# yeyupiaoling/PPASR

Hardware: AMD Instinct MI355X
Metric: audio-seconds/s (RTF^-1) Conformer-streaming fbank, batch32 per GPU, ctc_greedy (higher is better)
Workload: dtype f32; 1 GPU; configs[1]: Conformer streaming (configs/conformer.yml), fbank-80, 32 x 10 s utterances per GPU, V=4233, ctc_greedy, features resident in HBM -> token ids + scores on device; global_batch=32, frames=1000, decoder=ctc_greedy, parallelism=utterance-dp1, pipelined=False, gemm=f32

## Files before the change

### ppasr_amd/csrc/conformer_kernels.hip

```cpp
#include <cstdlib>

#include "conformer_kernels.h"
#include "launch.h"
#include "phases.h"
#include "h3.h"

#include <math.h>

namespace ppasr {
#ifdef PPASR_PHASE_TS
}
extern "C" __attribute__((visibility("default"))) int ppasr_debug_read_phase_ts(long long* out) {
  return (int)hipMemcpyFromSymbol(out, HIP_SYMBOL(ppasr::g_phase_ts), sizeof(long long) * 128);
}
extern "C" __attribute__((visibility("default"))) int ppasr_debug_read_wave_ts(long long* out) {
  return (int)hipMemcpyFromSymbol(out, HIP_SYMBOL(ppasr::g_wave_ts), sizeof(long long) * 512);
}
extern "C" __attribute__((visibility("default"))) int ppasr_debug_read_wg_ts(long long* out) {
  return (int)hipMemcpyFromSymbol(out, HIP_SYMBOL(ppasr::g_wg_ts), sizeof(long long) * 2 * 1024);
}
namespace ppasr {
#endif


// ... 281 lines not shown
    }
    const float bval = w.pw1_b[col];
    const float bgate = w.pw1_b[kD + col];
#pragma unroll
    for (int r = 0; r < 16; ++r) {
      int row = acc_row(r, lane);
      float val = av[0][0][r] + bval;
      float gate = ag[0][0][r] + bgate;
      if (row < valid) g[(size_t)(r0 + row) * kD + col] = val * sigmoidf(gate);
    }
  }
}
template <bool H3>
__global__ __launch_bounds__(kThreads) void k_pw1_glu_cols(const float* __restrict__ xhat, float* __restrict__ g, LayerW w,
                                                           int M, PadSkip ps) {
  extern __shared__ __attribute__((aligned(16))) float smem[];
  const int blk = pad_block_of(ps, kRows, M);
  if (blk < 0) return;
  float* bufA = smem;
  float* vals = bufA + kRows * kLda + (H3 ? 128 : 0);
  const int lane = lane_id(), wave = wave_id();
  const int r0 = blk * kRows;
  const int valid = min(kRows, M - r0);
  const int is_gate = wave >> 2, t = wave & 3, y = blockIdx.y;
  const int col = 128 * y + 32 * t + (lane & 31);
  const f32x4* seg = w.pw1 + (size_t)((is_gate ? 8 : 0) + 4 * y + t) * kTs256;
  BRing<1> ring;
  ring_prime(ring, seg, 0);
  rb_load_rows(bufA, kLda, xhat + (size_t)r0 * kD, kRows, valid);
  __syncthreads();
  f32x16 acc[1][1];
  acc_zero(acc);
  if constexpr (H3) unit_std_h3(bufA, seg, nullptr, ring, acc);
  else rb_gemm<1, 1, kG256>(bufA, kLda, seg, 0, nullptr, 0, ring, acc);
  const float bv = w.pw1_b[(is_gate ? kD : 0) + col];
  if (!is_gate) {
#pragma unroll
    for (int r = 0; r < 16; ++r) vals[acc_row(r, lane) * 132 + 32 * t + (lane & 31)] = acc[0][0][r] + bv;
  }
  __syncthreads();
  if (is_gate) {
#pragma unroll
    for (int r = 0; r < 16; ++r) {
      const int row = acc_row(r, lane);
      if (row < valid) g[(size_t)(r0 + row) * kD + col] = vals[row * 132 + 32 * t + (lane & 31)] * sigmoidf(acc[0][0][r] + bv);
    }
  }
}
constexpr size_t kLdsOutGlu = 2 * kRows * kLda * sizeof(float);
constexpr size_t kLdsPw1Cols = (kRows * kLda + kRows * 132) * sizeof(float);
void launch_out_glu(const float* ctx, const float* x1, float* x2, float* g, float* xhat_out, const LayerW& w,
                    const int64_t* lens, int M, int Tp, int mask_mul, hipStream_t st, const PadSkip& ps, float* split_xhat,
                    bool h3, HistMove* hm, int rows) {
  check_form("launch_out_glu", rows, h3 || xhat_out || split_xhat || hm);
  if (rows == 16) return LayerStagesT<16>::out_glu(ctx, x1, x2, g, w, lens, M, Tp, mask_mul, st, ps);
  if (rows == kW16) return LayerStagesT<kW16>::out_glu(ctx, x1, x2, g, w, lens, M, Tp, mask_mul, st, ps);
  float* xh = xhat_out ? xhat_out : split_xhat;
  if (split_xhat && !h3 && M <= kSplitRows16Max && !ps.tab) {
    const bool move = hm && hm->hist && hm->lo > 0 && hm->lo <= 30;
    launch_out_glu_split_16(ctx, x1, x2, g, xh, w, lens, M, Tp, mask_mul, st, ps, move ? hm->hist : nullptr, move ? hm->lo : 0);
    if (move) hm->done = true;
    return;
  }
  const dim3 grid((M + kRows - 1) / kRows);
  if (h3)
    PPASR_LAUNCH(k_out_glu<true>, grid, dim3(kThreads), kLdsOutGlu + 512, st, ctx, x1, x2, g, xh, w, lens, M, Tp, mask_mul, ps,
                 split_xhat ? 1 : 0);
  else
    PPASR_LAUNCH(k_out_glu<false>, grid, dim3(kThreads), kLdsOutGlu, st, ctx, x1, x2, g, xh, w, lens, M, Tp, mask_mul, ps,
                 split_xhat ? 1 : 0);
  if (split_xhat) {
    if (h3)
      PPASR_LAUNCH(k_pw1_glu_cols<true>, dim3(grid.x, 2), dim3(kThreads), kLdsPw1Cols + 512, st, xh, g, w, M, ps);
    else
      PPASR_LAUNCH(k_pw1_glu_cols<false>, dim3(grid.x, 2), dim3(kThreads), kLdsPw1Cols, st, xh, g, w, M, ps);
  }
}

constexpr int kPLd = 68;
constexpr int kPTile = 32 * kPLd;
constexpr int kFusedAttnFloats = kWaves * kPTile + kWaves * 64 + kRows * kLda;
static_assert(2 * kRows * kLda <= kWaves * kPTile + kWaves * 64, "bufX/bufA alias the attention scratch");
static_assert(kRows * kLda + 128 + 4 * kPTile <= kWaves * kPTile, "the d rows (fp16 x3: the Q'_v planes, 512 B longer) and the four merge tiles fit in front of Stat");
static_assert(kH3TileBytes <= kRows * kLda * 4 + 512, "fp16 x3: the Q'_u planes at bufC run 512 B past it (the launch asks for them)");
static_assert(kRows * kLda * 4 + kH3TileBytes <= kWaves * kPTile * 4, "fp16 x3: operand planes at bufA stay in front of Stat");
static_assert(kFusedAttnFloats * 4 <= 160 * 1024, "LDS budget");
template <bool H3>
__device__ __forceinline__ void attn_out_glu_body(const AttnArgs& a, int B, const float* __restrict__ x1, float* __restrict__ x2,
                                                  float* __restrict__ g, const LayerW& w) {
  extern __shared__ __attribute__((aligned(16))) float smem[];
  float* Ps = smem;
  float* Stat = Ps + kWaves * kPTile;
  float* bufC = Stat + kWaves * 64;
  float* bufX = smem;
  float* bufA = bufX + kRows * kLda;
  const int lane = lane_id(), wave = wave_id();
  const int h = wave >> 1, khalf = wave & 1;
  const int nq = (a.T1 + 31) / 32;
  const int slot = blockIdx.x >> 3;
  const int b = (slot / nq) * 8 + (blockIdx.x & 7);
  const int q0 = (slot % nq) * 32;
  if (b >= B) return;
  const int T = a.T1;
  const int valid = min(32, T - q0);
  const float* __restrict__ qb = a.q + (size_t)b * T * a.q_stride;
  const float* __restrict__ kbp = a.k + (size_t)b * a.T2 * a.k_stride;
  const float* __restrict__ vbp = a.v + (size_t)b * a.T2 * a.v_stride;
  const float* __restrict__ ptab = a.ptab + (size_t)a.pos0 * kD;
  const int pstride = a.pos_stride;
  const int64_t len_b = a.lens ? a.lens[b] : (int64_t)a.mask_mul * a.T2;
  int T2 = a.T2;
  if (a.pad_skip > 0 && a.lens) {
    const int64_t lb = len_b > 0 ? len_b : 0;
    const int64_t n_valid = (lb + a.mask_mul - 1) / a.mask_mul;
    if (q0 >= min((int64_t)T, n_valid + (a.pad_skip - 1))) return;
    T2 = (int)max((int64_t)1, min((int64_t)T2, n_valid));
  }
  float* QV = Ps;
  float* P = Ps + kRows * kLda + (H3 ? 128 : 0) + (wave >> 1) * kPTile;
  BRing<1> ring;
  const f32x4* seg_o = w.wo + (size_t)wave * kTs256;
  const f32x4* seg_val = w.pw1 + (size_t)wave * kTs256;
  const f32x4* seg_gate = w.pw1 + (size_t)(8 + wave) * kTs256;
  const int hh = lane >> 5, l31 = lane & 31;
  constexpr int NG = H3 ? 16 : 8;
  PPASR_TS(32);
  PPASR_WG_TS(512 + 0);

  const int mrow0 = b * T;
  const int shift = mrow0 & 7;
  int kv_end = (int)min((int64_t)T2, max((int64_t)0, (len_b + a.mask_mul - 1) / a.mask_mul));
  const int U = kv_end > 0 ? kv_end + shift : 0;
  constexpr float kScale = 0.125f * 1.4426950408889634f * (H3 ? 1.0f / (kH3Sa * kH3Sa) : 1.0f);
  const __amdgpu_buffer_rsrc_t rs_k = wstream_rsrc(kbp + h * (H3 ? 32 : 64)), rs_p = wstream_rsrc(ptab + h * (H3 ? 32 : 64)),
                               rs_v = wstream_rsrc(a.vt + ((size_t)(2 * h) * (a.vt_stride >> 3) + ((mrow0 - shift) >> 3)) * 256);
  const int voff_v = lane * 16;
  const int kstride_b = a.k_stride * 4, pstride_b = pstride * kD * 4;
  int vk[2], vp[2];
  auto key_offsets = [&](int u0) {
#pragma unroll
    for (int t = 0; t < 2; ++t) {
      const int key = min(max(u0 - shift + 32 * t + l31, 0), kv_end - 1);
      vk[t] = key * kstride_b + 16 * hh;
      if constexpr (H3) vp[t] = key * pstride_b + 16 * hh;
    }
  };
  constexpr int NKB = H3 ? 4 : 2;
  f32x4 kq[NKB][4][2];
  auto load_sg = [&](int buf, int sg) {
#pragma unroll
    for (int i = 0; i < 4; ++i) {
      if constexpr (H3) {
        const int soff = (sg & 1) * 512 + 32 * i;
        kq[buf][i][0] = sg < 2 ? wstream_load(rs_k, vk[0], soff) : wstream_load(rs_p, vp[0], soff);
        kq[buf][i][1] = sg < 2 ? wstream_load(rs_k, vk[1], soff) : wstream_load(rs_p, vp[1], soff);
      } else {
        kq[buf][i][0] = wstream_load(rs_k, vk[0], (4 * sg + i) * 32);
        kq[buf][i][1] = wstream_load(rs_k, vk[1], (4 * sg + i) * 32);
      }
    }
  };
  auto prime_k = [&](int u0) {
    key_offsets(u0);
    load_sg(0, 0);
    if constexpr (H3) load_sg(1, 1);
  };

  const float* __restrict__ dtab = a.dtab ? a.dtab + (size_t)h * a.dtab_len + a.pos0 : nullptr;
  {
    if constexpr (!H3) attn_stage_d(Ps + h * kDRow, dtab, khalf * 64 + lane, shift, U <= kDRow ? U : 0, pstride);
    const f32x4 pu = *reinterpret_cast<const f32x4*>(a.pos_u + 4 * lane), pv = *reinterpret_cast<const f32x4*>(a.pos_v + 4 * lane);
    bool bad = false;
    for (int row = wave; row < kRows; row += kWaves) {
      f32x4 v = {0.f, 0.f, 0.f, 0.f};
      if (row < valid) v = *reinterpret_cast<const f32x4*>(qb + (size_t)(q0 + row) * a.q_stride + 4 * lane);
      if constexpr (H3) {
        f16x4 hi, lo;
        h3_split4((v + pu) * kH3Sa, hi, lo, bad);
        _Float16* pu_pl = reinterpret_cast<_Float16*>(bufC) + row * kLdh + 4 * lane;
        *reinterpret_cast<f16x4*>(pu_pl) = hi;
        *reinterpret_cast<f16x4*>(pu_pl + kPlaneH) = lo;
        h3_split4((v + pv) * kH3Sa, hi, lo, bad);
        _Float16* pv_pl = reinterpret_cast<_Float16*>(QV) + row * kLdh + 4 * lane;
        *reinterpret_cast<f16x4*>(pv_pl) = hi;
        *reinterpret_cast<f16x4*>(pv_pl + kPlaneH) = lo;
      } else {
        *reinterpret_cast<f32x4*>(bufC + row * kLda + 4 * lane) = v + pu;
      }
    }
    if constexpr (H3) h3_note(bad);
    __syncthreads();
  }
  const float* qfrag_u = bufC + l31 * kLda + h * 64 + 4 * hh;
  auto qfrag = [&](int gk) -> f32x4 { return *reinterpret_cast<const f32x4*>(qfrag_u + 8 * gk); };
  PPASR_TS(33);
  if (khalf * 128 < U) prime_k(khalf * 128);
  f32x16 acc_o[2];
#pragma unroll
  for (int t = 0; t < 2; ++t)
#pragma unroll
    for (int r = 0; r < 16; ++r) acc_o[t][r] = 0.f;
  float m_run = -INFINITY, l_run = 0.f;
  bool first = true;

  const int nkb = (U + 255) / 256;
  for (int kb = 0; kb < nkb; ++kb) {
    for (int sb = 0; sb < 2; ++sb) {
      const int u0 = kb * 256 + khalf * 128 + sb * 64;
      if (u0 >= U) break;
      int u_next = sb == 0 ? u0 + 64 : (kb + 1) * 256 + khalf * 128;
      if (u_next >= U) u_next = (sb == 0 && (kb + 1) * 256 + khalf * 128 < U) ? (kb + 1) * 256 + khalf * 128 : -1;
      const bool edge = (u0 < shift) || (u0 + 64 > U);
      if (kb == 0) PPASR_WAVE_TS(16 + 4 * sb);
      const int soff_v = (u0 >> 3) * 1024, soff_v1 = soff_v + (a.vt_stride >> 3) * 1024;
      auto vload = [&](int q, int ct) -> f32x4 { return wstream_load(rs_v, voff_v, (ct ? soff_v1 : soff_v) + q * 1024); };
      constexpr int PQ = 8;
      f32x4 ringv[PQ][2];
      auto prime_v = [&]() {
#pragma unroll
        for (int q = 0; q < PQ; ++q) {
          ringv[q][0] = vload(q, 0);
          ringv[q][1] = vload(q, 1);
        }
      };
      f32x16 acc_s[2];
      if constexpr (H3) {
#pragma unroll
        for (int t = 0; t < 2; ++t)
#pragma unroll
          for (int r = 0; r < 16; ++r) acc_s[t][r] = 0.f;
      } else {
        attn_score_init(acc_s, U <= kDRow ? Ps + h * kDRow + u0 + 4 * hh : nullptr, dtab, u0 - shift + 4 * hh, kv_end, pstride);
      }
      if constexpr (H3) {
        const _Float16* qu = reinterpret_cast<const _Float16*>(bufC) + l31 * kLdh + h * 64 + 8 * hh;
        const _Float16* qv = reinterpret_cast<const _Float16*>(QV) + l31 * kLdh + h * 64 + 8 * hh;
        load_sg(2, 2);
        load_sg(3, 3);
#pragma unroll
        for (int sg = 0; sg < 4; ++sg) {
          const _Float16* qp = sg < 2 ? qu : qv;
#pragma unroll
          for (int i = 0; i < 4; ++i) {
            const f16x8 qh = *reinterpret_cast<const f16x8*>(qp + 16 * i);
            const f16x8 k0 = __builtin_bit_cast(f16x8, kq[sg][i][0]), k1 = __builtin_bit_cast(f16x8, kq[sg][i][1]);
            if ((sg & 1) == 0) {
              const f16x8 ql = *reinterpret_cast<const f16x8*>(qp + kPlaneH + 16 * i);
              acc_s[0] = __builtin_amdgcn_mfma_f32_32x32x16_f16(k0, ql, acc_s[0], 0, 0, 0);
              acc_s[1] = __builtin_amdgcn_mfma_f32_32x32x16_f16(k1, ql, acc_s[1], 0, 0, 0);
            }
            acc_s[0] = __builtin_amdgcn_mfma_f32_32x32x16_f16(k0, qh, acc_s[0], 0, 0, 0);
            acc_s[1] = __builtin_amdgcn_mfma_f32_32x32x16_f16(k1, qh, acc_s[1], 0, 0, 0);
            __builtin_amdgcn_sched_barrier(0);
          }
        }
      } else {
        f32x4 q_cur = qfrag(0), q_nxt = q_cur;
#pragma unroll
        for (int sg = 0; sg < 2; ++sg) {
          if (sg == 0) load_sg(1, 1);
#pragma unroll
          for (int i = 0; i < 4; ++i) {
            const int gk = 4 * sg + i;
            if (gk + 1 < NG) q_nxt = qfrag(gk + 1);
            const f32x4 k0 = kq[sg][i][0], k1 = kq[sg][i][1];
#pragma unroll
            for (int j = 0; j < 4; ++j) {
              acc_s[0] = __builtin_amdgcn_mfma_f32_32x32x2f32(k0[j], q_cur[j], acc_s[0], 0, 0, 0);
              acc_s[1] = __builtin_amdgcn_mfma_f32_32x32x2f32(k1[j], q_cur[j], acc_s[1], 0, 0, 0);
            }
            q_cur = q_nxt;
            __builtin_amdgcn_sched_barrier(0);
          }
        }
      }
      if (kb == 0) PPASR_WAVE_TS(17 + 4 * sb);
      prime_v();
      if (edge) {
        const int lo = shift - u0 - 4 * hh, hi = U - u0 - 4 * hh;
        if (u0 < shift) {
#pragma unroll
          for (int r = 0; r < 4; ++r)
            if (r < lo) acc_s[0][r] = -INFINITY;
        }
        if (u0 + 64 > U) {
#pragma unroll
          for (int t = 0; t < 2; ++t)
#pragma unroll
            for (int r = 0; r < 16; ++r)
              if (32 * t + (r & 3) + 8 * (r >> 2) >= hi) acc_s[t][r] = -INFINITY;
        }
      }
      float bm = max3f(acc_s[0][0], acc_s[0][1], acc_s[0][2]);
#pragma unroll
      for (int r = 3; r < 15; r += 2) bm = max3f(bm, acc_s[0][r], acc_s[0][r + 1]);
      bm = max3f(bm, acc_s[0][15], acc_s[1][0]);
#pragma unroll
      for (int r = 1; r < 15; r += 2) bm = max3f(bm, acc_s[1][r], acc_s[1][r + 1]);
      bm = fmaxf(bm, acc_s[1][15]);
      bm = fmaxf(bm, __shfl_xor(bm, 32));
      const float m_new = fmaxf(m_run, bm);
      const float m_safe = (m_new == -INFINITY) ? 0.f : m_new;
      const float alpha = __builtin_amdgcn_exp2f((m_run - m_safe) * kScale);
      const float mb = -m_safe * kScale;
      f32x2 ps2 = {0.f, 0.f};
#pragma unroll
      for (int t = 0; t < 2; ++t)
#pragma unroll
        for (int r = 0; r < 16; r += 2) {
          const f32x2 e = f32x2{acc_s[t][r], acc_s[t][r + 1]} * f32x2{kScale, kScale} + f32x2{mb, mb};
          acc_s[t][r] = __builtin_amdgcn_exp2f(e[0]);
          acc_s[t][r + 1] = __builtin_amdgcn_exp2f(e[1]);
          ps2 += f32x2{acc_s[t][r], acc_s[t][r + 1]};
        }
      float ps = ps2[0] + ps2[1];
      ps += __shfl_xor(ps, 32);
      m_run = m_new;
      l_run = l_run * alpha + ps;
      if (u_next >= 0) prime_k(u_next);
      if (kb == 0) PPASR_WAVE_TS(18 + 4 * sb);
      if (!first) {
#pragma unroll
        for (int ct = 0; ct < 2; ++ct)
#pragma unroll
          for (int r = 0; r < 16; r += 2) {
            const f32x2 o = f32x2{acc_o[ct][r], acc_o[ct][r + 1]} * f32x2{alpha, alpha};
            acc_o[ct][r] = o[0];
            acc_o[ct][r + 1] = o[1];
          }
      }
      first = false;
#pragma unroll
      for (int q = 0; q < 8; ++q) {
        const f32x4 v0 = ringv[q][0], v1 = ringv[q][1];
#pragma unroll
        for (int j = 0; j < 4; ++j) {
          const float pj = acc_s[q >> 2][4 * (q & 3) + j];
          acc_o[0] = __builtin_amdgcn_mfma_f32_32x32x2f32(v0[j], pj, acc_o[0], 0, 0, 0);
          acc_o[1] = __builtin_amdgcn_mfma_f32_32x32x2f32(v1[j], pj, acc_o[1], 0, 0, 0);
        }
        __builtin_amdgcn_sched_barrier(0);
      }
      if (kb == 0) PPASR_WAVE_TS(19 + 4 * sb);
    }
  }
  PPASR_TS(34);
  if (khalf == 1) {
    if (hh == 0) {
      Stat[wave * 64 + l31] = m_run;
      Stat[wave * 64 + 32 + l31] = l_run;
    }
#pragma unroll
    for (int ct = 0; ct < 2; ++ct)
#pragma unroll
      for (int i = 0; i < 4; ++i)
        *reinterpret_cast<f32x4*>(P + l31 * kPLd + 32 * ct + 8 * i + 4 * hh) =
            f32x4{acc_o[ct][4 * i], acc_o[ct][4 * i + 1], acc_o[ct][4 * i + 2], acc_o[ct][4 * i + 3]};
  }
  const int r0 = b * T + q0;
  const int cq = wave * 32 + 4 * hh;
  const size_t grow = (size_t)(r0 + min(l31, valid - 1)) * kD;
  const bool row_ok = l31 < valid;
  f32x4 res[4];
  if constexpr (H3) {
#pragma unroll
    for (int q = 0; q < 4; ++q) res[q] = *reinterpret_cast<const f32x4*>(x1 + grow + cq + 8 * q);
  }
  ring_prime(ring, seg_o, 0);
  __syncthreads();
  PPASR_TS(35);
  if (khalf == 0) {
    const float* P1 = P;
    const float m1 = Stat[(wave + 1) * 64 + l31], l1 = Stat[(wave + 1) * 64 + 32 + l31];
    const float m = fmaxf(m_run, m1);
    const float e0 = (m_run == -INFINITY) ? 0.f : __builtin_amdgcn_exp2f((m_run - m) * kScale);
    const float e1 = (m1 == -INFINITY) ? 0.f : __builtin_amdgcn_exp2f((m1 - m) * kScale);
    const float l = l_run * e0 + l1 * e1;
    float inv = (l > 0.f) ? 1.0f / l : 0.f;
    if (l31 >= valid) inv = 0.f;
    const float f0 = e0 * inv, f1 = e1 * inv;
#pragma unroll
    for (int ct = 0; ct < 2; ++ct)
#pragma unroll
      for (int i = 0; i < 4; ++i) {
        const f32x4 o1 = *reinterpret_cast<const f32x4*>(P1 + l31 * kPLd + 32 * ct + 8 * i + 4 * hh);
        f32x4 o;
#pragma unroll
        for (int e = 0; e < 4; ++e) o[e] = acc_o[ct][4 * i + e] * f0 + o1[e] * f1;
        *reinterpret_cast<f32x4*>(bufC + l31 * kLda + h * 64 + 32 * ct + 8 * i + 4 * hh) = o;
      }
  }
  __syncthreads();
  PPASR_TS(36);
  f32x4 x2v[4];
  {
    if constexpr (!H3) {
#pragma unroll
      for (int q = 0; q < 4; ++q) res[q] = *reinterpret_cast<const f32x4*>(x1 + grow + cq + 8 * q);
    }
    f32x16 acc[1][1];
    acc_zero(acc);
    if constexpr (H3) {
      h3_planes_from_tile(bufC, reinterpret_cast<_Float16*>(bufA));
      rb_gemm_h3(reinterpret_cast<const _Float16*>(bufA), seg_o, seg_val, ring, acc[0][0]);
      acc[0][0] *= kH3Inv;
    } else {
      rb_gemm<1, 1, kG256, kPF, NoSide, true>(bufC, kLda, seg_o, 0, seg_val, 0, ring, acc);
    }
#pragma unroll
    for (int q = 0; q < 4; ++q) {
      const f32x4 bo = *reinterpret_cast<const f32x4*>(w.bo + cq + 8 * q);
      f32x4 v;
#pragma unroll
      for (int e = 0; e < 4; ++e) v[e] = res[q][e] + (acc[0][0][4 * q + e] + bo[e]);
      if constexpr (H3) x2v[q] = v;
      else if (row_ok) *reinterpret_cast<f32x4*>(x2 + grow + cq + 8 * q) = v;
      if (!row_ok) v = f32x4{0.f, 0.f, 0.f, 0.f};
      *reinterpret_cast<f32x4*>(bufX + l31 * kLda + cq + 8 * q) = v;
    }
  }
  __syncthreads();
  PPASR_TS(37);
  struct PadHere {
    int64_t len_b;
    int q0, mul;
    __device__ __forceinline__ bool operator()(int row) const { return (int64_t)mul * (q0 + row) >= len_b; }
  };
  rb_layernorm<false>(bufX, bufA, kLda, kRows, w.ln_conv_g, w.ln_conv_b, 1e-5f,
                      PadHere{a.lens ? len_b : (int64_t)1 << 62, q0, a.mask_mul});
  __syncthreads();
  PPASR_TS(38);
  {
    f32x16 av[1][1], ag[1][1];
    acc_zero(av);
    acc_zero(ag);
    if constexpr (H3) {
      h3_planes_from_tile(bufA, reinterpret_cast<_Float16*>(bufA));
      rb_gemm_h3(reinterpret_cast<const _Float16*>(bufA), seg_val, seg_gate, ring, av[0][0]);
      rb_gemm_h3(reinterpret_cast<const _Float16*>(bufA), seg_gate, nullptr, ring, ag[0][0]);
      av[0][0] *= kH3Inv;
      ag[0][0] *= kH3Inv;
    } else {
      rb_gemm<1, 1, kG256, kPF, NoSide, true>(bufA, kLda, seg_val, 0, seg_gate, 0, ring, av);
      rb_gemm<1, 1, kG256, kPF, NoSide, true>(bufA, kLda, seg_gate, 0, nullptr, 0, ring, ag);
    }
#pragma unroll
    for (int q = 0; q < 4; ++q) {
      const f32x4 bval = *reinterpret_cast<const f32x4*>(w.pw1_b + cq + 8 * q);
      const f32x4 bgate = *reinterpret_cast<const f32x4*>(w.pw1_b + kD + cq + 8 * q);
      const f32x2 s0 = sigmoid2(f32x2{ag[0][0][4 * q] + bgate[0], ag[0][0][4 * q + 1] + bgate[1]});
      const f32x2 s1 = sigmoid2(f32x2{ag[0][0][4 * q + 2] + bgate[2], ag[0][0][4 * q + 3] + bgate[3]});
      const f32x4 o = {(av[0][0][4 * q] + bval[0]) * s0[0], (av[0][0][4 * q + 1] + bval[1]) * s0[1],
                       (av[0][0][4 * q + 2] + bval[2]) * s1[0], (av[0][0][4 * q + 3] + bval[3]) * s1[1]};
      if (row_ok) *reinterpret_cast<f32x4*>(g + grow + cq + 8 * q) = o;
// ... 339 lines not shown
```

### ppasr_amd/csrc/phases.h

```cpp
#pragma once
#include "conformer_kernels.h"
#include "rowblock.h"

namespace ppasr {

struct SwishSide {
  const f32x16& acc;
  float* dst;
  const f32x4 (&bias)[4];
  mutable f32x2 lo;
  __device__ __forceinline__ void operator()(int g) const {
    const int q = g >> 3;
    if ((g & 7) == 0) lo = swish2(f32x2{acc[4 * q] + bias[q][0], acc[4 * q + 1] + bias[q][1]});
    if ((g & 7) == 4) {
      const f32x2 hi = swish2(f32x2{acc[4 * q + 2] + bias[q][2], acc[4 * q + 3] + bias[q][3]});
      *reinterpret_cast<f32x4*>(dst + 8 * q) = f32x4{lo[0], lo[1], hi[0], hi[1]};
    }
  }
};

template <bool T2 = false>
__device__ __forceinline__ void ffn_phase(const float* bufA, float* bufH, const f32x4* __restrict__ w1,
                                          const float* __restrict__ b1, const f32x4* __restrict__ w2, int n_chunks,
                                          const f32x4* __restrict__ after, BRing<1>& ring, f32x16 (&acc2)[1][1],
// ... 113 lines not shown
        if (tt < 0 && m < M) xv = *reinterpret_cast<const f32x4*>(hist + (size_t)(LO + tt) * kD);
      } else if (!(tt >= 0 && tt < Tp)) {
        xv = gp;
      }
      acc += wj * xv;
    }
    *reinterpret_cast<f32x4*>(bufA + row * kLda + 4 * lane) = acc;
  }
}

template <int KS>
__device__ __forceinline__ void dwconv_ln_phase(const float* __restrict__ g, float* bufA, const float* __restrict__ dw_w,
                                                const float* __restrict__ dw_b, const float* __restrict__ glu_pad,
                                                const float* __restrict__ ln_g, const float* __restrict__ ln_b, float ln_eps, int r0,
                                                int M, int Tp, int left) {
  const int lane = lane_id(), wave = wave_id();
  constexpr int LO = KS - 1, RW = kRows / kWaves, NW = RW + LO;
  const bool causal = (left == LO);
  const int q0 = wave * RW;
  f32x4 x[NW];
#pragma unroll
  for (int q = 0; q < NW; ++q) {
    const int mq = r0 - left + q0 + q;
    const int mc = min(max(mq, 0), M - 1);
    const f32x4 v = *reinterpret_cast<const f32x4*>(g + (size_t)mc * kD + 4 * lane);
    x[q] = (mq >= 0 && mq < M) ? v : f32x4{0.f, 0.f, 0.f, 0.f};
  }
  f32x4 wt[KS];
#pragma unroll
  for (int j = 0; j < KS; ++j) wt[j] = *reinterpret_cast<const f32x4*>(dw_w + j * kD + 4 * lane);
  f32x4 gp = *reinterpret_cast<const f32x4*>(glu_pad + 4 * lane);
  if (!causal) gp = f32x4{0.f, 0.f, 0.f, 0.f};
  const f32x4 bias = *reinterpret_cast<const f32x4*>(dw_b + 4 * lane);
  const int m0 = r0 + q0;
  const int tq0 = m0 - (m0 / Tp) * Tp;
  const int npass = (tq0 + RW - 1 < Tp) ? 1 : 2;
  f32x4 out[RW];
#pragma unroll 1
  for (int p = 0; p < npass; ++p) {
    const int tqp = tq0 - p * Tp;
    f32x4 acc[RW];
#pragma unroll
    for (int i = 0; i < RW; ++i) acc[i] = bias;
#pragma unroll
    for (int q = 0; q < NW; ++q) {
      const int tt = tqp - left + q;
      const f32x4 xq = (tt >= 0 && tt < Tp) ? x[q] : gp;
#pragma unroll
      for (int i = 0; i < RW; ++i) {
        const int j = q - i;
        if (j >= 0 && j < KS) acc[i] += wt[j] * xq;
      }
    }
#pragma unroll
    for (int i = 0; i < RW; ++i)
      if (npass == 1 || (tqp + i >= 0 && tqp + i < Tp)) out[i] = acc[i];
  }
  const f32x4 gam = *reinterpret_cast<const f32x4*>(ln_g + 4 * lane);
  const f32x4 bet = *reinterpret_cast<const f32x4*>(ln_b + 4 * lane);
  ln_rows_inreg<true, RW>(out, gam, bet, ln_eps);
#pragma unroll
  for (int i = 0; i < RW; ++i) *reinterpret_cast<f32x4*>(bufA + (q0 + i) * kLda + 4 * lane) = out[i];
}

template <bool H3>
__device__ __forceinline__ f32x4 qkv_bias_quad(const float* __restrict__ bqkv, const VtOut& vt, int c, int m, int col) {
  if (c < 2) return *reinterpret_cast<const f32x4*>(bqkv + c * 256 + col);
  if constexpr (!H3) {
    if (vt.kpos) return *reinterpret_cast<const f32x4*>(vt.kpos + (size_t)(m - m / vt.Ti * vt.Ti) * vt.kpos_stride + col);
  }
  return f32x4{0.f, 0.f, 0.f, 0.f};
}
template <bool H3>
__device__ __forceinline__ void qkv_kpos_add(f32x4 (&bk)[4], const f32x4 (&kp)[4], const VtOut& vt) {
  if constexpr (!H3) {
    if (vt.kpos) {
#pragma unroll
      for (int q = 0; q < 4; ++q) bk[q] += kp[q];
    }
  }
}
constexpr int kDRow = 2048;
static_assert(4 * kDRow <= kRows * kLda, "the four heads' d rows fit in front of the merge tiles");
__device__ __forceinline__ void attn_stage_d(float* row, const float* __restrict__ dtab, int t128, int shift, int U, int pstride) {
  for (int u = t128; u < ((U + 63) & ~63); u += 128)
    row[u] = (dtab && u >= shift && u < U) ? dtab[(size_t)(u - shift) * pstride] : 0.f;
}
__device__ __forceinline__ void attn_score_init(f32x16 (&acc_s)[2], const float* dl, const float* __restrict__ dtab, int key0,
                                                int kv_end, int pstride) {
#pragma unroll
  for (int t = 0; t < 2; ++t)
#pragma unroll
    for (int i = 0; i < 4; ++i) {
      f32x4 dq;
      if (dl) {
        dq = *reinterpret_cast<const f32x4*>(dl + 32 * t + 8 * i);
      } else {
#pragma unroll
        for (int j = 0; j < 4; ++j)
          dq[j] = dtab ? dtab[(size_t)min(max(key0 + 32 * t + 8 * i + j, 0), kv_end - 1) * pstride] : 0.f;
      }
#pragma unroll
      for (int j = 0; j < 4; ++j) acc_s[t][4 * i + j] = dq[j];
    }
}

}
```

### ppasr_amd/csrc/phases_t.h

```cpp
#pragma once
#include "phases.h"
#include "rbt.h"

namespace ppasr {

template <int R>
struct LaneT {
  int lane, wave;
  __device__ __forceinline__ LaneT() : lane(lane_id()), wave(wave_id()) {}
  __device__ __forceinline__ int row(int q) const { return RBT<R>::row(q, lane); }
  __device__ __forceinline__ int col(int q) const { return RBT<R>::col(q, lane, wave); }
  __device__ __forceinline__ int off(int q) const { return row(q) * kLda + col(q); }
  __device__ __forceinline__ int tile() const { return RBT<R>::tile(wave); }
  __device__ __forceinline__ int quads_ok(int valid) const {
    int n = 0;
#pragma unroll
    for (int q = 0; q < RBT<R>::NQ; ++q) n += row(q) < valid ? 1 : 0;
    return n;
  }
};

template <int R>
__device__ __forceinline__ void rbt_load_rows(float* dst, const float* __restrict__ src, int valid) {
  const int lane = lane_id();
// ... 119 lines not shown
    float* p = bufX + L.off(q);
    const f32x4 bv = *reinterpret_cast<const f32x4*>(bias + L.col(q));
    const f32x4 a = RBT<R>::quad(acc, q);
    f32x4 x = *reinterpret_cast<const f32x4*>(p);
#pragma unroll
    for (int e = 0; e < 4; ++e) x[e] = x[e] + scale * (a[e] + bv[e]);
    *reinterpret_cast<f32x4*>(p) = x;
  }
}

template <int R>
struct QuadStoreSide {
  const typename RBT<R>::Acc& acc;
  float* out;
  int qstep;
  int n_ok;
  const f32x4 (&bias)[RBT<R>::NQ];
  __device__ __forceinline__ void operator()(int g) const {
    constexpr int STEP = 32 / RBT<R>::NQ;
    const int q = g / STEP;
    if (g % STEP == STEP / 2 && q < n_ok) {
      const f32x4 v = RBT<R>::quad(acc, q);
      *reinterpret_cast<f32x4*>(out + q * qstep) = f32x4{v[0] + bias[q][0], v[1] + bias[q][1], v[2] + bias[q][2], v[3] + bias[q][3]};
    }
  }
};

template <int R>
__device__ __forceinline__ void qkv_phase_t(const float* bufX, float* __restrict__ qkv, const f32x4* __restrict__ wqkv,
                                            const float* __restrict__ bqkv, int r0, int valid, typename RBT<R>::Ring& ring,
                                            float* __restrict__ vt = nullptr, int vt_stride = 0,
                                            const float* __restrict__ kpos = nullptr, int kpos_stride = 0, int Ti = 1) {
  using T = RBT<R>;
  const LaneT<R> L;
  float* q0 = qkv + (size_t)(r0 + L.row(0)) * 768 + L.col(0);
  const int qs = T::qstep(768), n_ok = L.quads_ok(valid);
  f32x4 qb[3][T::NQ];
#pragma unroll
  for (int c = 0; c < 3; ++c)
#pragma unroll
    for (int q = 0; q < T::NQ; ++q) qb[c][q] = *reinterpret_cast<const f32x4*>(bqkv + c * 256 + L.col(q));
  if (kpos) {
#pragma unroll
    for (int q = 0; q < T::NQ; ++q) {
      const int m = r0 + L.row(q);
      qb[1][q] += *reinterpret_cast<const f32x4*>(kpos + (size_t)(m - m / Ti * Ti) * kpos_stride + L.col(q));
    }
  }
  typename T::Acc tile[3];
#pragma unroll
  for (int c = 0; c < 3; ++c) {
    T::zero(tile[c]);
    const f32x4* seg = wqkv + (size_t)(c * 8 + L.tile()) * kTs256;
    const f32x4* nseg = c < 2 ? seg + 8 * kTs256 : nullptr;
    if (c == 0) {
      rbt_gemm<kG256>(bufX, kLda, seg, nseg, ring, tile[c]);
    } else {
      const QuadStoreSide<R> store{tile[c - 1], q0 + (c - 1) * 256, qs, n_ok, qb[c - 1]};
      if constexpr (R == kW16) {
        if (c == 2 && vt) rbt_gemm<kG256, QuadStoreSide<R>, false>(bufX, kLda, seg, nseg, ring, tile[c], store);
        else rbt_gemm<kG256>(bufX, kLda, seg, nseg, ring, tile[c], store);
      } else {
        rbt_gemm<kG256>(bufX, kLda, seg, nseg, ring, tile[c], store);
      }
    }
  }
  if constexpr (R == kW16) {
    if (vt) {
      const int c32 = 16 * (L.wave & 1) + (L.lane & 15), kq = L.lane >> 4;
      const float bv = bqkv[512 + 16 * L.wave + (L.lane & 15)];
      float* dst = vt + ((size_t)(L.wave >> 1) * (vt_stride >> 3) + (r0 >> 3) + (kq >> 1)) * 256 + 4 * (c32 + 32 * (kq & 1));
#pragma unroll
      for (int q = 0; q < 2; ++q) {
        const f32x4 v = tile[2].s[q];
        *reinterpret_cast<f32x4*>(dst + q * 512) = f32x4{v[0] + bv, v[1] + bv, v[2] + bv, v[3] + bv};
      }
      return;
    }
  }
#pragma unroll
  for (int q = 0; q < T::NQ; ++q) {
    if (q < n_ok) *reinterpret_cast<f32x4*>(q0 + 512 + q * qs) = T::quad(tile[2], q) + qb[2][q];
  }
}

__device__ __forceinline__ __amdgpu_buffer_rsrc_t buf_rsrc(const void* p, size_t bytes) {
  const uint64_t a = reinterpret_cast<uint64_t>(p);
  const uint32_t lo = __builtin_amdgcn_readfirstlane((uint32_t)a), hi = __builtin_amdgcn_readfirstlane((uint32_t)(a >> 32));
  const uint32_t n = __builtin_amdgcn_readfirstlane((uint32_t)(bytes > 0xffffffffull ? 0xffffffffull : bytes));
  return __builtin_amdgcn_make_buffer_rsrc(reinterpret_cast<void*>(((uint64_t)hi << 32) | lo), 0, (int)n, 0x00020000);
}

template <int RW, int J0, int JN>
__device__ __forceinline__ void dw_chunk(__amdgpu_buffer_rsrc_t rs_g, __amdgpu_buffer_rsrc_t rs_w, f32x4 (&acc)[RW],
                                         const f32x4& gp, int mwin0, int tqp, int left, int Tp, int lane, int zero) {
  constexpr int NWC = JN + RW - 1;
  const int vrow = lane * 16 + (mwin0 + J0) * (kD * 4);
  f32x4 x[NWC];
#pragma unroll
  for (int qq = 0; qq < NWC; ++qq) x[qq] = wstream_load(rs_g, vrow + qq * (kD * 4), zero);
  f32x4 wt[JN];
#pragma unroll
  for (int j = 0; j < JN; ++j) wt[j] = wstream_load(rs_w, lane * 16, (J0 + j) * (kD * 4) + zero);
#pragma unroll
  for (int qq = 0; qq < NWC; ++qq) {
    const int tt = tqp - left + J0 + qq;
    if (!(tt >= 0 && tt < Tp)) x[qq] = gp;
#pragma unroll
    for (int i = 0; i < RW; ++i) {
      const int j = qq - i;
      if (j >= 0 && j < JN) acc[i] += wt[j] * x[qq];
    }
  }
}

template <int RW, int KS, int TC, int J0>
__device__ __forceinline__ void dw_chunks(__amdgpu_buffer_rsrc_t rs_g, __amdgpu_buffer_rsrc_t rs_w, f32x4 (&acc)[RW],
                                          const f32x4& gp, int mwin0, int tqp, int left, int Tp, int lane, int zero) {
  constexpr int JN = KS - J0 < TC ? KS - J0 : TC;
  dw_chunk<RW, J0, JN>(rs_g, rs_w, acc, gp, mwin0, tqp, left, Tp, lane, zero);
  if constexpr (J0 + JN < KS) {
#pragma unroll
    for (int i = 0; i < RW; ++i) asm volatile("" : "+v"(acc[i]));
    __builtin_amdgcn_sched_barrier(0);
    dw_chunks<RW, KS, TC, J0 + JN>(rs_g, rs_w, acc, gp, mwin0, tqp, left, Tp, lane, zero);
  }
}

template <int R, int KS, typename Between>
__device__ __forceinline__ void dwconv_ln_phase_t(const float* __restrict__ g, float* bufA, const float* __restrict__ dw_w,
                                                  const float* __restrict__ dw_b, const float* __restrict__ glu_pad,
                                                  const float* __restrict__ ln_g, const float* __restrict__ ln_b, float ln_eps,
                                                  int r0, int M, int Tp, int left, Between between) {
  const int lane = lane_id(), wave = wave_id();
  constexpr int LO = KS - 1, RW = RBT<R>::RW, TC = KS <= RBT<R>::DW_TC ? 16 : RBT<R>::DW_TC;
  const bool causal = (left == LO);
  const int q0 = wave * RW;
  f32x4 gp = *reinterpret_cast<const f32x4*>(glu_pad + 4 * lane);
  if (!causal) gp = f32x4{0.f, 0.f, 0.f, 0.f};
  const f32x4 bias = *reinterpret_cast<const f32x4*>(dw_b + 4 * lane);
  const int m0 = r0 + q0;
  const int tq0 = __builtin_amdgcn_readfirstlane(m0 - (m0 / Tp) * Tp);
  const int npass = (tq0 + RW - 1 < Tp) ? 1 : 2;
  const __amdgpu_buffer_rsrc_t rs_g = buf_rsrc(g, (size_t)M * kD * sizeof(float)), rs_w = wstream_rsrc(dw_w);
  f32x4 out[RW];
#pragma unroll 1
  for (int p = 0; p < npass; ++p) {
    int zero;
    asm volatile("s_mov_b32 %0, 0" : "=s"(zero));
    const int tqp = tq0 - p * Tp;
    f32x4 acc[RW];
#pragma unroll
    for (int i = 0; i < RW; ++i) acc[i] = bias;
    dw_chunks<RW, KS, TC, 0>(rs_g, rs_w, acc, gp, m0 - left, tqp, left, Tp, lane, zero);
#pragma unroll
    for (int i = 0; i < RW; ++i)
      if (npass == 1 || (tqp + i >= 0 && tqp + i < Tp)) out[i] = acc[i];
  }
  __builtin_amdgcn_sched_barrier(0);
  between();
  const f32x4 gam = *reinterpret_cast<const f32x4*>(ln_g + 4 * lane);
  const f32x4 bet = *reinterpret_cast<const f32x4*>(ln_b + 4 * lane);
  ln_rows_inreg<true, RW>(out, gam, bet, ln_eps);
#pragma unroll
  for (int i = 0; i < RW; ++i) *reinterpret_cast<f32x4*>(bufA + (q0 + i) * kLda + 4 * lane) = out[i];
}

}
```

Before: 58570 audio-s/s.

## Keep f32 attention Q in registers and merge halves symmetrically

In the fp32 fused attention path, each wave now loads its Q fragments plus pos_u straight into registers at kernel entry, ahead of the length checks. This drops the staging of Q through LDS and the barrier that followed it. The d-row staging is reworked as chunked buffer loads issued before the K prime, so those fetches overlap. The final split-K softmax merge is also made symmetric: both key halves hand over a tile and each merges half of the output columns, instead of one half idling. The cost is about 64 extra VGPRs per lane for qreg and pu, which may lower occupancy, plus a different LDS layout for the hand-over tiles.

Measured after the change: 58690 audio-s/s (median of 6 runs). About the same (+0.2%).

```diff
diff --git a/ppasr_amd/csrc/conformer_kernels.hip b/ppasr_amd/csrc/conformer_kernels.hip
--- a/ppasr_amd/csrc/conformer_kernels.hip
+++ b/ppasr_amd/csrc/conformer_kernels.hip
@@ -387,6 +387,7 @@
 constexpr int kFusedAttnFloats = kWaves * kPTile + kWaves * 64 + kRows * kLda;
 static_assert(2 * kRows * kLda <= kWaves * kPTile + kWaves * 64, "bufX/bufA alias the attention scratch");
 static_assert(kRows * kLda + 128 + 4 * kPTile <= kWaves * kPTile, "the d rows (fp16 x3: the Q'_v planes, 512 B longer) and the four merge tiles fit in front of Stat");
+static_assert(4 * kDRow + kWaves * kMTile <= kWaves * kPTile, "fp32: the d rows and the eight hand-over tiles fit in front of Stat");
 static_assert(kH3TileBytes <= kRows * kLda * 4 + 512, "fp16 x3: the Q'_u planes at bufC run 512 B past it (the launch asks for them)");
 static_assert(kRows * kLda * 4 + kH3TileBytes <= kWaves * kPTile * 4, "fp16 x3: operand planes at bufA stay in front of Stat");
 static_assert(kFusedAttnFloats * 4 <= 160 * 1024, "LDS budget");
@@ -413,6 +414,8 @@
   const float* __restrict__ vbp = a.v + (size_t)b * a.T2 * a.v_stride;
   const float* __restrict__ ptab = a.ptab + (size_t)a.pos0 * kD;
   const int pstride = a.pos_stride;
+  f32x4 qreg[8], pu[8];
+  if constexpr (!H3) attn_q_request(qreg, pu, qb + (size_t)q0 * a.q_stride, valid, a.q_stride, a.pos_u, h, lane);
   const int64_t len_b = a.lens ? a.lens[b] : (int64_t)a.mask_mul * a.T2;
   int T2 = a.T2;
   if (a.pad_skip > 0 && a.lens) {
@@ -428,7 +431,6 @@
   const f32x4* seg_val = w.pw1 + (size_t)wave * kTs256;
   const f32x4* seg_gate = w.pw1 + (size_t)(8 + wave) * kTs256;
   const int hh = lane >> 5, l31 = lane & 31;
-  constexpr int NG = H3 ? 16 : 8;
   PPASR_TS(32);
   PPASR_WG_TS(512 + 0);
 
@@ -472,34 +474,30 @@
   };
 
   const float* __restrict__ dtab = a.dtab ? a.dtab + (size_t)h * a.dtab_len + a.pos0 : nullptr;
-  {
-    if constexpr (!H3) attn_stage_d(Ps + h * kDRow, dtab, khalf * 64 + lane, shift, U <= kDRow ? U : 0, pstride);
+  if constexpr (H3) {
     const f32x4 pu = *reinterpret_cast<const f32x4*>(a.pos_u + 4 * lane), pv = *reinterpret_cast<const f32x4*>(a.pos_v + 4 * lane);
     bool bad = false;
     for (int row = wave; row < kRows; row += kWaves) {
       f32x4 v = {0.f, 0.f, 0.f, 0.f};
       if (row < valid) v = *reinterpret_cast<const f32x4*>(qb + (size_t)(q0 + row) * a.q_stride + 4 * lane);
-      if constexpr (H3) {
-        f16x4 hi, lo;
-        h3_split4((v + pu) * kH3Sa, hi, lo, bad);
-        _Float16* pu_pl = reinterpret_cast<_Float16*>(bufC) + row * kLdh + 4 * lane;
-        *reinterpret_cast<f16x4*>(pu_pl) = hi;
-        *reinterpret_cast<f16x4*>(pu_pl + kPlaneH) = lo;
-        h3_split4((v + pv) * kH3Sa, hi, lo, bad);
-        _Float16* pv_pl = reinterpret_cast<_Float16*>(QV) + row * kLdh + 4 * lane;
-        *reinterpret_cast<f16x4*>(pv_pl) = hi;
-        *reinterpret_cast<f16x4*>(pv_pl + kPlaneH) = lo;
-      } else {
-        *reinterpret_cast<f32x4*>(bufC + row * kLda + 4 * lane) = v + pu;
-      }
-    }
-    if constexpr (H3) h3_note(bad);
+      f16x4 hi, lo;
+      h3_split4((v + pu) * kH3Sa, hi, lo, bad);
+      _Float16* pu_pl = reinterpret_cast<_Float16*>(bufC) + row * kLdh + 4 * lane;
+      *reinterpret_cast<f16x4*>(pu_pl) = hi;
+      *reinterpret_cast<f16x4*>(pu_pl + kPlaneH) = lo;
+      h3_split4((v + pv) * kH3Sa, hi, lo, bad);
+      _Float16* pv_pl = reinterpret_cast<_Float16*>(QV) + row * kLdh + 4 * lane;
+      *reinterpret_cast<f16x4*>(pv_pl) = hi;
+      *reinterpret_cast<f16x4*>(pv_pl + kPlaneH) = lo;
+    }
+    h3_note(bad);
     __syncthreads();
-  }
-  const float* qfrag_u = bufC + l31 * kLda + h * 64 + 4 * hh;
-  auto qfrag = [&](int gk) -> f32x4 { return *reinterpret_cast<const f32x4*>(qfrag_u + 8 * gk); };
-  PPASR_TS(33);
-  if (khalf * 128 < U) prime_k(khalf * 128);
+    PPASR_TS(33);
+    if (khalf * 128 < U) prime_k(khalf * 128);
+  } else {
+    attn_prologue_f32(qreg, pu, Ps + h * kDRow, dtab, kv_end, pstride, shift, U, khalf, lane, [&] { if (khalf * 128 < U) prime_k(khalf * 128); });
+    PPASR_TS(33);
+  }
   f32x16 acc_o[2];
 #pragma unroll
   for (int t = 0; t < 2; ++t)
@@ -560,21 +558,17 @@
           }
         }
       } else {
-        f32x4 q_cur = qfrag(0), q_nxt = q_cur;
 #pragma unroll
         for (int sg = 0; sg < 2; ++sg) {
           if (sg == 0) load_sg(1, 1);
 #pragma unroll
           for (int i = 0; i < 4; ++i) {
-            const int gk = 4 * sg + i;
-            if (gk + 1 < NG) q_nxt = qfrag(gk + 1);
-            const f32x4 k0 = kq[sg][i][0], k1 = kq[sg][i][1];
+            const f32x4 k0 = kq[sg][i][0], k1 = kq[sg][i][1], qf = qreg[4 * sg + i];
 #pragma unroll
             for (int j = 0; j < 4; ++j) {
-              acc_s[0] = __builtin_amdgcn_mfma_f32_32x32x2f32(k0[j], q_cur[j], acc_s[0], 0, 0, 0);
-              acc_s[1] = __builtin_amdgcn_mfma_f32_32x32x2f32(k1[j], q_cur[j], acc_s[1], 0, 0, 0);
+              acc_s[0] = __builtin_amdgcn_mfma_f32_32x32x2f32(k0[j], qf[j], acc_s[0], 0, 0, 0);
+              acc_s[1] = __builtin_amdgcn_mfma_f32_32x32x2f32(k1[j], qf[j], acc_s[1], 0, 0, 0);
             }
-            q_cur = q_nxt;
             __builtin_amdgcn_sched_barrier(0);
           }
         }
@@ -650,7 +644,9 @@
     }
   }
   PPASR_TS(34);
-  if (khalf == 1) {
+  float* Pm = Ps + 4 * kDRow + wave * kMTile;
+  if constexpr (!H3) attn_hand_over_f32(Stat, Pm, wave, acc_o, m_run, l_run, l31, hh);
+  else if (khalf == 1) {
     if (hh == 0) {
       Stat[wave * 64 + l31] = m_run;
       Stat[wave * 64 + 32 + l31] = l_run;
@@ -674,7 +670,9 @@
   ring_prime(ring, seg_o, 0);
   __syncthreads();
   PPASR_TS(35);
-  if (khalf == 0) {
+  if constexpr (!H3) {
+    attn_merge_f32(bufC + l31 * kLda + h * 64 + 4 * hh, Stat, Pm, wave, acc_o, m_run, l_run, kScale, l31 < valid, l31, hh);
+  } else if (khalf == 0) {
     const float* P1 = P;
     const float m1 = Stat[(wave + 1) * 64 + l31], l1 = Stat[(wave + 1) * 64 + 32 + l31];
     const float m = fmaxf(m_run, m1);
diff --git a/ppasr_amd/csrc/phases.h b/ppasr_amd/csrc/phases.h
--- a/ppasr_amd/csrc/phases.h
+++ b/ppasr_amd/csrc/phases.h
@@ -219,9 +219,105 @@
 }
 constexpr int kDRow = 2048;
 static_assert(4 * kDRow <= kRows * kLda, "the four heads' d rows fit in front of the merge tiles");
-__device__ __forceinline__ void attn_stage_d(float* row, const float* __restrict__ dtab, int t128, int shift, int U, int pstride) {
-  for (int u = t128; u < ((U + 63) & ~63); u += 128)
-    row[u] = (dtab && u >= shift && u < U) ? dtab[(size_t)(u - shift) * pstride] : 0.f;
+__device__ __forceinline__ __amdgpu_buffer_rsrc_t buf_rsrc(const void* p, size_t bytes) {
+  const uint64_t a = reinterpret_cast<uint64_t>(p);
+  const uint32_t lo = __builtin_amdgcn_readfirstlane((uint32_t)a), hi = __builtin_amdgcn_readfirstlane((uint32_t)(a >> 32));
+  const uint32_t n = __builtin_amdgcn_readfirstlane((uint32_t)(bytes > 0xffffffffull ? 0xffffffffull : bytes));
+  return __builtin_amdgcn_make_buffer_rsrc(reinterpret_cast<void*>(((uint64_t)hi << 32) | lo), 0, (int)n, 0x00020000);
+}
+constexpr int kDChunk = 4;
+__device__ __forceinline__ __amdgpu_buffer_rsrc_t attn_d_rsrc(const float* __restrict__ dtab, int kv_end, int pstride) {
+  return buf_rsrc(dtab, dtab && kv_end > 0 ? ((size_t)(kv_end - 1) * pstride + 1) * sizeof(float) : 0);
+}
+__device__ __forceinline__ int attn_d_key(int kb, int j, int khalf, int lane) { return 256 * (kb + (j >> 1)) + 128 * khalf + 64 * (j & 1) + lane; }
+__device__ __forceinline__ void attn_d_request(float (&dv)[2 * kDChunk], __amdgpu_buffer_rsrc_t rs_d, int kb, int khalf, int lane,
+                                               int shift, int pstride) {
+#pragma unroll
+  for (int j = 0; j < 2 * kDChunk; ++j)
+    dv[j] = __builtin_bit_cast(float, __builtin_amdgcn_raw_buffer_load_b32(rs_d, (attn_d_key(kb, j, khalf, lane) - shift) * pstride * 4, 0, 0));
+}
+__device__ __forceinline__ void attn_d_store(float* row, const float (&dv)[2 * kDChunk], int kb, int khalf, int lane, int U) {
+#pragma unroll
+  for (int j = 0; j < 2 * kDChunk; ++j) {
+    const int u = attn_d_key(kb, j, khalf, lane);
+    if (u < ((U + 63) & ~63)) row[u] = dv[j];
+  }
+}
+template <class PrimeK>
+__device__ __forceinline__ void attn_prologue_f32(f32x4 (&qreg)[8], const f32x4 (&pu)[8], float* drow, const float* __restrict__ dtab,
+                                                  int kv_end, int pstride, int shift, int U, int khalf, int lane, PrimeK prime_k) {
+  const int nkb_d = U <= kDRow ? (U + 255) / 256 : 0;
+  const __amdgpu_buffer_rsrc_t rs_d = attn_d_rsrc(dtab, kv_end, pstride);
+  float dv[2 * kDChunk];
+  if (nkb_d > 0) attn_d_request(dv, rs_d, 0, khalf, lane, shift, pstride);
+  prime_k();
+#pragma unroll
+  for (int gk = 0; gk < 8; ++gk) qreg[gk] = qreg[gk] + pu[gk];
+  if (nkb_d > 0) attn_d_store(drow, dv, 0, khalf, lane, U);
+  for (int kb = kDChunk; kb < nkb_d; kb += kDChunk) {
+    attn_d_request(dv, rs_d, kb, khalf, lane, shift, pstride);
+    attn_d_store(drow, dv, kb, khalf, lane, U);
+  }
+  __builtin_amdgcn_fence(__ATOMIC_ACQ_REL, "wavefront");
+}
+__device__ __forceinline__ void attn_q_request(f32x4 (&qreg)[8], f32x4 (&pu)[8], const float* __restrict__ qrows, int valid,
+                                               int q_stride, const float* __restrict__ pos_u, int h, int lane) {
+  const __amdgpu_buffer_rsrc_t rs_q = buf_rsrc(qrows, ((size_t)(valid - 1) * q_stride + kD) * sizeof(float)),
+                               rs_u = wstream_rsrc(pos_u);
+  const int voff_u = 16 * (lane >> 5), voff_q = (lane & 31) * q_stride * 4 + voff_u;
+#pragma unroll
+  for (int gk = 0; gk < 8; ++gk) qreg[gk] = wstream_load(rs_q, voff_q, 256 * h + 32 * gk);
+#pragma unroll
+  for (int gk = 0; gk < 8; ++gk) pu[gk] = wstream_load(rs_u, voff_u, 256 * h + 32 * gk);
+}
+constexpr int kMLd = 36;
+constexpr int kMTile = 32 * kMLd;
+__device__ __forceinline__ void attn_hand_over(float* tile, const f32x16& o, int l31, int hh) {
+#pragma unroll
+  for (int i = 0; i < 4; ++i)
+    *reinterpret_cast<f32x4*>(tile + l31 * kMLd + 8 * i + 4 * hh) = f32x4{o[4 * i], o[4 * i + 1], o[4 * i + 2], o[4 * i + 3]};
+}
+__device__ __forceinline__ void attn_hand_over_f32(float* stat, float* tile, int wave, const f32x16 (&acc_o)[2], float m_run, float l_run,
+                                                   int l31, int hh) {
+  if (hh == 0) {
+    stat[wave * 64 + l31] = m_run;
+    stat[wave * 64 + 32 + l31] = l_run;
+  }
+  if (wave & 1) attn_hand_over(tile, acc_o[0], l31, hh);
+  else attn_hand_over(tile, acc_o[1], l31, hh);
+}
+__device__ __forceinline__ void attn_merge_factors(float m0, float l0, float m1, float l1, float scale, bool keep, float& f0, float& f1) {
+  const float m = fmaxf(m0, m1);
+  const float e0 = (m0 == -INFINITY) ? 0.f : __builtin_amdgcn_exp2f((m0 - m) * scale);
+  const float e1 = (m1 == -INFINITY) ? 0.f : __builtin_amdgcn_exp2f((m1 - m) * scale);
+  const float l = __builtin_fmaf(l0, e0, l1 * e1);
+  float inv = (l > 0.f) ? 1.0f / l : 0.f;
+  if (!keep) inv = 0.f;
+  f0 = e0 * inv;
+  f1 = e1 * inv;
+}
+template <int CT>
+__device__ __forceinline__ void attn_merge_half(float* dst, const float* other, const f32x16& own, float f0, float f1, int l31, int hh) {
+#pragma unroll
+  for (int i = 0; i < 4; ++i) {
+    const f32x4 ot = *reinterpret_cast<const f32x4*>(other + l31 * kMLd + 8 * i + 4 * hh);
+    f32x4 o;
+#pragma unroll
+    for (int e = 0; e < 4; ++e) {
+      const float o0 = CT == 0 ? own[4 * i + e] : ot[e], o1 = CT == 0 ? ot[e] : own[4 * i + e];
+      o[e] = (CT == 0 || i == 0) ? __builtin_fmaf(o1, f1, o0 * f0) : __builtin_fmaf(o0, f0, o1 * f1);
+    }
+    *reinterpret_cast<f32x4*>(dst + 8 * i) = o;
+  }
+}
+__device__ __forceinline__ void attn_merge_f32(float* crow, const float* stat, const float* tile, int wave, const f32x16 (&acc_o)[2],
+                                               float m_run, float l_run, float scale, bool keep, int l31, int hh) {
+  const int khalf = wave & 1;
+  const float mo = stat[(wave ^ 1) * 64 + l31], lo = stat[(wave ^ 1) * 64 + 32 + l31];
+  float f0, f1;
+  attn_merge_factors(khalf ? mo : m_run, khalf ? lo : l_run, khalf ? m_run : mo, khalf ? l_run : lo, scale, keep, f0, f1);
+  if (khalf == 0) attn_merge_half<0>(crow, tile + kMTile, acc_o[0], f0, f1, l31, hh);
+  else attn_merge_half<1>(crow + 32, tile - kMTile, acc_o[1], f0, f1, l31, hh);
 }
 __device__ __forceinline__ void attn_score_init(f32x16 (&acc_s)[2], const float* dl, const float* __restrict__ dtab, int key0,
                                                 int kv_end, int pstride) {
diff --git a/ppasr_amd/csrc/phases_t.h b/ppasr_amd/csrc/phases_t.h
--- a/ppasr_amd/csrc/phases_t.h
+++ b/ppasr_amd/csrc/phases_t.h
@@ -225,13 +225,6 @@
   for (int q = 0; q < T::NQ; ++q) {
     if (q < n_ok) *reinterpret_cast<f32x4*>(q0 + 512 + q * qs) = T::quad(tile[2], q) + qb[2][q];
   }
-}
-
-__device__ __forceinline__ __amdgpu_buffer_rsrc_t buf_rsrc(const void* p, size_t bytes) {
-  const uint64_t a = reinterpret_cast<uint64_t>(p);
-  const uint32_t lo = __builtin_amdgcn_readfirstlane((uint32_t)a), hi = __builtin_amdgcn_readfirstlane((uint32_t)(a >> 32));
-  const uint32_t n = __builtin_amdgcn_readfirstlane((uint32_t)(bytes > 0xffffffffull ? 0xffffffffull : bytes));
-  return __builtin_amdgcn_make_buffer_rsrc(reinterpret_cast<void*>(((uint64_t)hi << 32) | lo), 0, (int)n, 0x00020000);
 }
 
 template <int RW, int J0, int JN>
```
